# BattleZips/BattleZips-Halo2

Measured on AMD Instinct MI355X. Metric: complete proofs per second (synthesis + create_proof), BoardCircuit, k=14, IPA/Pasta, higher is better.
Workload: dtype u32x8 (255-bit modular integer, Montgomery)

## Files before the change

### battlezips-halo2_amd/bzh2/__init__.py

```python
from __future__ import annotations

import ctypes
import os

import numpy as np

_PKG = os.path.dirname(os.path.abspath(__file__))
_LIB_PATH = os.path.join(os.path.dirname(_PKG), "libbzh2.so")

OK, E_ARG, E_OOM, E_HIP, E_RANGE, E_NOGPU = 0, -1, -2, -3, -4, -5
CURVE_VESTA, CURVE_PALLAS, CURVE_BN254 = 0, 1, 2
FIELD_FP, FIELD_FQ, FIELD_BN254_FR, FIELD_BN254_FQ = 0, 1, 2, 3
FORM_CANONICAL, FORM_MONTGOMERY = 0, 1
MEM_HOST, MEM_DEVICE = 0, 1
T_MSM_DIGITS, T_MSM_ACCUMULATE, T_MSM_REDUCE, T_MSM_FINALIZE, T_NTT, T_COUNT = 0, 1, 2, 3, 4, 8
TIMER_NAMES = {0: "msm_digits", 1: "msm_accumulate", 2: "msm_reduce", 3: "msm_finalize", 4: "ntt"}

CURVE_SCALAR_FIELD = {CURVE_VESTA: FIELD_FP, CURVE_PALLAS: FIELD_FQ, CURVE_BN254: FIELD_BN254_FR}

EXPORTS = [
    "bzh_version", "bzh_strerror", "bzh_device_count", "bzh_ctx_create", "bzh_ctx_create_on_stream",
    "bzh_ctx_destroy", "bzh_ctx_sync", "bzh_last_error", "bzh_ctx_profile", "bzh_ctx_timings", "bzh_ctx_work", "bzh_ctx_msm_additions",
    "bzh_bases_upload", "bzh_bases_precompute", "bzh_bases_free", "bzh_bases_len", "bzh_bases_walk", "bzh_bases_points", "bzh_msm", "bzh_ntt", "bzh_coeff_to_extended",
    "bzh_jacobian_to_affine", "bzh_jacobian_sum", "bzh_affine_compress", "bzh_field_omega",
# ... 439 lines not shown
    out = np.zeros((v.shape[0], half, 4), dtype=np.uint64)
    _bind_poly(load())
    rc = load().bzh_fold(self.handle, field, _vp(v), half, v.shape[0], _vp(u), u.shape[0], form, MEM_HOST, _vp(out))
    self._check(rc, "bzh_fold")
    return out


def _ctx_vec_mul(self, field: int, a, b, form: int = FORM_CANONICAL) -> np.ndarray:
    a, b = _as_elems(a).copy(), _as_elems(b)
    _bind_poly(load())
    self._check(load().bzh_vec_mul(self.handle, field, _vp(a), _vp(b), a.size // 4, form, MEM_HOST), "bzh_vec_mul")
    return a


Context.batch_invert = _ctx_batch_invert
Context.prefix_product = _ctx_prefix_product
Context.eval_polynomial = _ctx_eval_polynomial
Context.inner_product = _ctx_inner_product
Context.fold = _ctx_fold
Context.vec_mul = _ctx_vec_mul


EXPORTS += ["bzh_pk_quotient_select", "bzh_pk_quotient_selected", "bzh_quotient_source_for_circuit", "bzh_builtin_quotients",
            "bzh_quotient_degree_histogram", "bzh_pk_lookup_select", "bzh_pk_lookup_selected"]
EXPORTS += ["bzh_record_stride", "bzh_record_encode", "bzh_record_decode", "bzh_record_to_json", "bzh_record_from_json"]
EXPORTS += ["bzh_transcript_new", "bzh_transcript_free", "bzh_transcript_common_point", "bzh_transcript_common_scalar",
            "bzh_transcript_write_point", "bzh_transcript_write_scalar", "bzh_transcript_squeeze_challenge",
            "bzh_transcript_proof"]


class Transcript:

    def __init__(self, challenge_field: int = FIELD_FP):
        L = load()
        vp = ctypes.c_void_p
        L.bzh_transcript_new.argtypes = [ctypes.c_int, ctypes.POINTER(vp)]
        for f in ("bzh_transcript_free",):
            getattr(L, f).argtypes = [vp]
        for f in ("bzh_transcript_common_point", "bzh_transcript_common_scalar", "bzh_transcript_write_scalar",
                  "bzh_transcript_squeeze_challenge"):
            getattr(L, f).argtypes = [vp, ctypes.POINTER(ctypes.c_uint64)]
        L.bzh_transcript_write_point.argtypes = [vp, ctypes.c_int, ctypes.POINTER(ctypes.c_uint64)]
        L.bzh_transcript_proof.argtypes = [vp, ctypes.POINTER(ctypes.POINTER(ctypes.c_uint8)), ctypes.POINTER(ctypes.c_size_t)]
        self.h = vp()
        rc = L.bzh_transcript_new(challenge_field, ctypes.byref(self.h))
        if rc != OK:
            raise BzhError(rc, "bzh_transcript_new")
# ... 262 lines not shown
```

### battlezips-halo2_amd/bzh2/native.py

```python
from __future__ import annotations

import ctypes

import numpy as np

from . import CURVE_SCALAR_FIELD, FORM_CANONICAL, FORM_MONTGOMERY, MEM_DEVICE, MEM_HOST, Bases, BzhError, Context, int_to_limbs, load
from .circuit_data import MODULI, Circuit, serialize_circuit

_VP = ctypes.c_void_p


def _bind():
    L = load()
    if getattr(L, "_bzh_native_bound", False):
        return L
    L.bzh_pk_create.argtypes = [_VP, _VP, ctypes.c_char_p, ctypes.c_size_t, ctypes.POINTER(_VP)]
    L.bzh_pk_free.argtypes = [_VP, _VP]
    L.bzh_pk_set_lagrange.argtypes = [_VP, _VP]
    L.bzh_pk_info.argtypes = [_VP, ctypes.POINTER(ctypes.c_size_t), ctypes.POINTER(ctypes.c_size_t), ctypes.POINTER(ctypes.c_uint32),
                              ctypes.POINTER(ctypes.c_uint32), ctypes.POINTER(ctypes.c_uint32)]
    L.bzh_verify_batch.argtypes = [_VP, _VP, ctypes.c_size_t, _VP, ctypes.c_size_t, _VP, ctypes.c_size_t, ctypes.POINTER(ctypes.c_size_t), _VP,
                                   ctypes.POINTER(ctypes.c_int)]
    L.bzh_prove_batch.argtypes = [_VP, _VP, ctypes.c_size_t, _VP, ctypes.c_int, ctypes.c_int, _VP, ctypes.c_size_t, ctypes.c_char_p,
                                  ctypes.c_size_t, _VP, ctypes.c_size_t, ctypes.POINTER(ctypes.c_size_t)]
# ... 100 lines not shown
                                                          np.concatenate([int_to_limbs(wp[0]), int_to_limbs(wp[1])])]))
        blob = bytes(circuit) if isinstance(circuit, (bytes, bytearray)) else serialize_circuit(circuit, self.p, vk_repr)
        L = _bind()
        h = _VP()
        ctx._check(L.bzh_pk_create(ctx.handle, self.bases.handle, blob, len(blob), ctypes.byref(h)), "bzh_pk_create")
        self.handle = h
        rb, mp = ctypes.c_size_t(), ctypes.c_size_t()
        na, nr, ur = ctypes.c_uint32(), ctypes.c_uint32(), ctypes.c_uint32()
        ctx._check(L.bzh_pk_info(h, ctypes.byref(rb), ctypes.byref(mp), ctypes.byref(na), ctypes.byref(nr), ctypes.byref(ur)), "bzh_pk_info")
        self.rng_bytes, self.max_proof_bytes, self.num_advice, self.n, self.usable_rows = rb.value, mp.value, na.value, nr.value, ur.value
        if params is not None:
            self.set_lagrange(params.bases_lagrange)

    def vk_repr(self):
        out, ph = (ctypes.c_uint8 * 32)(), ctypes.c_int()
        self.ctx._check(_bind().bzh_pk_vk_repr(self.handle, out, ctypes.byref(ph)), "bzh_pk_vk_repr")
        return int.from_bytes(bytes(out), "little"), bool(ph.value)

    def quotient_stats(self) -> dict:
        L = _bind()
        L.bzh_pk_quotient_stats.argtypes = [_VP] + [ctypes.POINTER(ctypes.c_uint32)] * 4
        v = [ctypes.c_uint32() for _ in range(4)]
        self.ctx._check(L.bzh_pk_quotient_stats(self.handle, *[ctypes.byref(x) for x in v]), "bzh_pk_quotient_stats")
        return {"ops": v[0].value, "multiplications_per_row": v[1].value, "lds_slots": v[2].value, "hoisted_columns": v[3].value}

    def quotient_source(self) -> str:
        L = _bind()
        L.bzh_pk_quotient_source.argtypes = [_VP, ctypes.c_char_p, ctypes.c_size_t, ctypes.POINTER(ctypes.c_size_t)]
        n = ctypes.c_size_t()
        self.ctx._check(L.bzh_pk_quotient_source(self.handle, None, 0, ctypes.byref(n)), "bzh_pk_quotient_source")
        buf = ctypes.create_string_buffer(n.value + 1)
        self.ctx._check(L.bzh_pk_quotient_source(self.handle, buf, n.value + 1, ctypes.byref(n)), "bzh_pk_quotient_source")
        return buf.value.decode()

    def set_quotient_module(self, code_object: bytes | None):
        L = _bind()
        L.bzh_pk_set_quotient_module.argtypes = [_VP, _VP, ctypes.c_char_p, ctypes.c_size_t]
        self.ctx._check(L.bzh_pk_set_quotient_module(self.ctx.handle, self.handle, code_object, len(code_object) if code_object else 0),
                        "bzh_pk_set_quotient_module")

    def quotient_selected(self):
        L = _bind()
        L.bzh_pk_quotient_selected.argtypes = [_VP, ctypes.POINTER(ctypes.c_int), ctypes.POINTER(ctypes.c_int)]
        f, b = ctypes.c_int(), ctypes.c_int()
        self.ctx._check(L.bzh_pk_quotient_selected(self.handle, ctypes.byref(f), ctypes.byref(b)), "bzh_pk_quotient_selected")
        return f.value, bool(b.value)

# ... 205 lines not shown
```

### battlezips-halo2_amd/csrc/exprvm.hip

```cpp
#include "ctx.hpp"
#include "field.cuh"
#include "host_field.hpp"

namespace bzh {

static constexpr int kExprSlots = 24;

struct ExprOp {
    uint8_t op, dst, a_kind, b_kind;
    int32_t a_idx, b_idx, a_rot, b_rot;
};

template <class P>
__device__ __forceinline__ Fe<P> expr_operand(int kind, int idx, int rot, const Fe<P>* slots, const uint32_t* const* cols,
                                               const size_t* strides, const uint32_t* consts, size_t r, size_t mask, size_t v) {
    if (kind == BZH_EXPR_SLOT) return slots[idx];
    if (kind == BZH_EXPR_CONST) return fe_load<P>(consts + (size_t)idx * 8);
    const size_t row = (r + (size_t)(int64_t)rot) & mask;
    return fe_load<P>(cols[idx] + (v * strides[idx] + row) * 8);
}

template <class P>
__global__ void __launch_bounds__(256) k_expr_eval(const ExprOp* __restrict__ prog, int nops, const uint32_t* const* __restrict__ cols,
                                                     const size_t* __restrict__ strides, const uint32_t* __restrict__ consts,
// ... 86 lines not shown
    else
        hipLaunchKernelGGL((k_expr_eval<P>), grid, block, 0, ctx->stream, d_prog, nops, d_cols, d_strides, d_consts, const_stride, size,
                           result_slot, d_out);
    BZH_HIP_TRY(ctx, hipGetLastError());
    return BZH_OK;
}

int expr_eval(bzh_ctx* ctx, int field, const void* d_prog, int nops, const uint32_t* const* d_cols, const size_t* d_strides,
              const uint32_t* d_consts, size_t const_stride, size_t size, int result_slot, size_t batch, int nslots, uint32_t* d_out) {
    const ExprOp* p = (const ExprOp*)d_prog;
    return with_field(field, [&](auto f) {
        return expr_eval_t<decltype(f)>(ctx, p, nops, d_cols, d_strides, d_consts, const_stride, size, result_slot, batch, nslots, d_out);
    });
}


struct ExprOp2 {
    uint8_t code, a_kind, b_kind, pad;
    int32_t a_idx, b_idx;
    int16_t a_rot, b_rot;
};
static_assert(sizeof(ExprOp2) == 16, "ExprOp2 layout");

static constexpr int kVm2Threads = 128;

template <class P>
__global__ void __launch_bounds__(kVm2Threads) k_expr_vm2(const ExprOp2* __restrict__ prog, int nops, const uint32_t* const* __restrict__ cols,
                                                           const size_t* __restrict__ strides, const uint32_t* __restrict__ consts,
                                                           size_t const_stride, size_t size, uint32_t* __restrict__ out) {
    extern __shared__ uint4 vm2_lds[];
    const size_t r = blockIdx.x * (size_t)kVm2Threads + threadIdx.x, v = blockIdx.y;
    if (r >= size) return;
    const size_t mask = size - 1;
    const uint32_t* cv = consts + v * const_stride * 8;
    const unsigned t = threadIdx.x;
    Fe<P> r0 = fe_zero<P>(), r1 = r0, r2 = r0, r3 = r0;
    auto leaf = [&](int kind, int idx, int rot) -> Fe<P> {
        if (kind == BZH_EXPR_COLUMN) {
            const size_t row = (r + (size_t)(int64_t)rot) & mask;
            return fe_load<P>(cols[idx] + (v * strides[idx] + row) * 8);
        }
        if (kind == BZH_EXPR_CONST) return fe_load<P>(cv + (size_t)idx * 8);
        Fe<P> x;
        const uint4 lo = vm2_lds[((size_t)idx * 2) * kVm2Threads + t], hi = vm2_lds[((size_t)idx * 2 + 1) * kVm2Threads + t];
        x.l[0] = lo.x, x.l[1] = lo.y, x.l[2] = lo.z, x.l[3] = lo.w, x.l[4] = hi.x, x.l[5] = hi.y, x.l[6] = hi.z, x.l[7] = hi.w;
        return x;
    };
    auto store = [&](int idx, const Fe<P>& x) {
        vm2_lds[((size_t)idx * 2) * kVm2Threads + t] = make_uint4(x.l[0], x.l[1], x.l[2], x.l[3]);
        vm2_lds[((size_t)idx * 2 + 1) * kVm2Threads + t] = make_uint4(x.l[4], x.l[5], x.l[6], x.l[7]);
    };
#define VM2_ARITH(OP, A, B) ((OP) == 0 ? fe_add(A, B) : ((OP) == 1 ? fe_sub(A, B) : ((OP) == 2 ? fe_mul(A, B) : fe_sub(B, A))))
#define VM2_SS(OP, P0, RA, RB) case (0 << 4) | ((OP) << 2) | (P0): RA = VM2_ARITH(OP, RA, RB); break;
#define VM2_SL(OP, P0, RA)     case (1 << 4) | ((OP) << 2) | (P0): { const Fe<P> b_ = leaf(op.b_kind, op.b_idx, op.b_rot); RA = VM2_ARITH(OP, RA, b_); } break;
#define VM2_LL(OP, P0, RA)     case (2 << 4) | ((OP) << 2) | (P0): { const Fe<P> a_ = leaf(op.a_kind, op.a_idx, op.a_rot); const Fe<P> b_ = leaf(op.b_kind, op.b_idx, op.b_rot); RA = VM2_ARITH(OP, a_, b_); } break;
#define VM2_ALLOPS_SS(P0, RA, RB) VM2_SS(0, P0, RA, RB) VM2_SS(1, P0, RA, RB) VM2_SS(2, P0, RA, RB) VM2_SS(3, P0, RA, RB)
#define VM2_ALLOPS_SL(P0, RA) VM2_SL(0, P0, RA) VM2_SL(1, P0, RA) VM2_SL(2, P0, RA) VM2_SL(3, P0, RA)
#define VM2_ALLOPS_LL(P0, RA) VM2_LL(0, P0, RA) VM2_LL(1, P0, RA) VM2_LL(2, P0, RA)
#define VM2_UN(P0, RA)                                                                                   \
    case (3 << 4) | (0 << 2) | (P0): RA = fe_neg(RA); break;                                              \
    case (3 << 4) | (1 << 2) | (P0): RA = leaf(op.a_kind, op.a_idx, op.a_rot); break;                     \
    case (3 << 4) | (2 << 2) | (P0): store(op.a_idx, RA); break;
    ExprOp2 nxt = prog[0];
    for (int i = 0; i < nops; i++) {
        const ExprOp2 op = nxt;
        nxt = prog[i + 1 < nops ? i + 1 : i];
        switch (op.code) {
            VM2_ALLOPS_SS(0, r0, r1) VM2_ALLOPS_SS(1, r1, r2) VM2_ALLOPS_SS(2, r2, r3)
            VM2_ALLOPS_SL(0, r0) VM2_ALLOPS_SL(1, r1) VM2_ALLOPS_SL(2, r2) VM2_ALLOPS_SL(3, r3)
            VM2_ALLOPS_LL(0, r0) VM2_ALLOPS_LL(1, r1) VM2_ALLOPS_LL(2, r2) VM2_ALLOPS_LL(3, r3)
            VM2_UN(0, r0) VM2_UN(1, r1) VM2_UN(2, r2) VM2_UN(3, r3)
            default: break;
        }
    }
#undef VM2_UN
#undef VM2_ALLOPS_LL
#undef VM2_ALLOPS_SL
#undef VM2_ALLOPS_SS
#undef VM2_LL
#undef VM2_SL
#undef VM2_SS
#undef VM2_ARITH
    fe_store(out + (v * size + r) * 8, r0);
}

int expr_eval2(bzh_ctx* ctx, int field, const void* d_prog, int nops, const uint32_t* const* d_cols, const size_t* d_strides,
               const uint32_t* d_consts, size_t const_stride, size_t size, size_t batch, int nlds, uint32_t* d_out) {
    if (size % kVm2Threads) return BZH_E_ARG;
    const size_t lds = (size_t)std::max(nlds, 1) * 2 * kVm2Threads * sizeof(uint4);
    if (lds > 64 * 1024) return BZH_E_RANGE;
    ScopedTimer t(ctx, BZH_T_QUOTIENT);
    const dim3 grid((unsigned)(size / kVm2Threads), (unsigned)batch), block(kVm2Threads);
    const ExprOp2* p = (const ExprOp2*)d_prog;
    BZH_TRY(with_pasta_field(field, [&](auto f) {
        hipLaunchKernelGGL((k_expr_vm2<decltype(f)>), grid, block, lds, ctx->stream, p, nops, d_cols, d_strides, d_consts, const_stride, size, d_out);
        return BZH_OK;
    }));
    BZH_HIP_TRY(ctx, hipGetLastError());
    return BZH_OK;
}

int expr_slots() { return kExprSlots; }

}
```

### battlezips-halo2_amd/csrc/prove.hip

```cpp
#include <algorithm>
#include <chrono>
#include <cstdio>
#include <cstdlib>
#include <cstring>
#include <map>
#include <set>
#include <memory>
#include <string>
#include <thread>
#include <vector>

#include "chacha.hpp"
#include "ctx.hpp"
#include "curve.cuh"
#include "fe29.cuh"
#include "host_field.hpp"

extern "C" const bzh_builtin_quotient* bzh_builtin_quotients(size_t* count) __attribute__((weak));

#include "prove_kernels.cuh"
#include "key_shape.hpp"
#include "quotient_program.hpp"
#include "proving_key.hpp"
#include "verifying_key.hpp"
// ... 163 lines not shown
    if (!pk) return BZH_E_ARG;
    if (g_lagrange && ((g_lagrange->n != pk->n + 2 && g_lagrange->n != pk->n + 3) || g_lagrange->curve != pk->curve || g_lagrange->device != pk->device || !g_lagrange->pre_c))
        return BZH_E_ARG;
    std::lock_guard<std::mutex> lk(pk->mu);
    pk->srs_lagrange = g_lagrange;
    return BZH_OK;
}

int bzh_pk_quotient_stats(bzh_pk* pk, uint32_t* ops, uint32_t* multiplications, uint32_t* lds_slots, uint32_t* hoisted_columns) {
    if (!pk) return BZH_E_ARG;
    uint32_t no = 0, nm = 0, nl = 0;
    if (pk->q_ok) {
        no = (uint32_t)pk->qprog.ops.size();
        nl = (uint32_t)pk->qprog.nlds;
        for (auto& o : pk->qprog.ops) nm += ((o.code >> 4) < 3 && ((o.code >> 2) & 3) == bzh::V2_MUL);
    }
    if (ops) *ops = no;
    if (multiplications) *multiplications = nm;
    if (lds_slots) *lds_slots = nl;
    if (hoisted_columns) *hoisted_columns = (uint32_t)pk->hoist_cols;
    return BZH_OK;
}

static int copy_text(const std::string& src, char* buf, size_t cap, size_t* len) {
    *len = src.size();
    if (buf && cap) {
        const size_t n = std::min(cap - 1, src.size());
        memcpy(buf, src.data(), n);
        buf[n] = 0;
    }
    return BZH_OK;
}

int bzh_pk_quotient_source(bzh_pk* pk, char* buf, size_t cap, size_t* len) {
    if (!pk || !len) return BZH_E_ARG;
    if (!pk->q_ok) return BZH_E_RANGE;
    return copy_text(bzh::program2_source(pk->qprog, pk->field), buf, cap, len);
}

int bzh_quotient_source_for_circuit(int curve, const uint8_t* circuit, size_t circuit_len, char* buf, size_t cap, size_t* len,
                                    uint64_t* program_hash) {
    if (!circuit || !len) return BZH_E_ARG;
    bzh_pk pk;
    BZH_TRY(bzh::with_pasta_curve(curve, [&](auto c) {
        using C = decltype(c);
        bzh::ParsedKey<typename bzh::CurveInfo<C>::SF> po;
        return bzh::pk_parse_t<C>(circuit, circuit_len, pk, po);
    }));
    if (!pk.q_ok) return BZH_E_RANGE;
    if (program_hash) *program_hash = pk.q_hash;
    return copy_text(bzh::program2_source(pk.qprog, pk.field, true) + "\n" + bzh::program2_source29(pk.qprog, pk.field), buf, cap, len);
}

int bzh_quotient_degree_histogram(int curve, const uint8_t* circuit, size_t circuit_len, uint32_t* polys, uint32_t* muls) {
    if (!circuit || !polys || !muls) return BZH_E_ARG;
    return bzh::with_pasta_curve(curve, [&](auto c) { return quotient_histogram_t<decltype(c)>(circuit, circuit_len, polys, muls); });
}

int bzh_pk_quotient_select(bzh_pk* pk, int flavour) {
    if (!pk) return BZH_E_ARG;
    std::lock_guard<std::mutex> lk(pk->mu);
    switch (flavour) {
        case BZH_QUOTIENT_INTERPRETER: break;
        case BZH_QUOTIENT_BUILTIN:
            if (!pk->q_builtin) return BZH_E_RANGE;
            break;
        case BZH_QUOTIENT_MODULE:
            if (!pk->q_fn) return BZH_E_RANGE;
            break;
        default: return BZH_E_ARG;
    }
    pk->q_select = flavour;
    return BZH_OK;
}
// ... 241 lines not shown
```

### battlezips-halo2_amd/csrc/quotient_program.hpp

```cpp
#pragma once
enum { EX_CONST, EX_SYMBOL, EX_QUERY, EX_NEG, EX_ADD, EX_MUL, EX_SCALE };
struct ENode {
    uint8_t tag;
    int32_t col = 0, rot = 0;
    uint32_t val[8] = {0};
    int a = -1, b = -1;
};
enum { SY_THETA, SY_BETA, SY_GAMMA, SY_Y, SY_XN, SY_X1, SY_X2, SY_X4, SY_BD0  };

struct ConstEnt {
    int sym = -1;
    uint32_t val[8] = {0};
};
struct Program {
    std::vector<bzh_expr_op> ops;
    std::vector<ConstEnt> consts;
    int result_slot = 0;
};

struct EPool {
    std::vector<ENode> n;
    struct NodeKey {
        uint8_t tag;
        int32_t col, rot, a, b;
// ... 147 lines not shown
            a = operand(e.a);
        } else {
            a = operand(e.a);
            b = operand(e.b);
        }
        const int d = a.release >= 0 ? a.release : (b.release >= 0 ? b.release : alloc());
        push(e.tag == EX_ADD ? BZH_EXPR_ADD : BZH_EXPR_MUL, d, a, b);
        if (a.release >= 0 && a.release != d) free_slots.push_back(a.release);
        if (b.release >= 0 && b.release != d) free_slots.push_back(b.release);
        return d;
    }
};


struct ExprOp2 {
    uint8_t code, a_kind, b_kind, pad;
    int32_t a_idx, b_idx;
    int16_t a_rot, b_rot;
};
enum { BZH_EXPR_LDS = 3 };
enum { V2_ADD = 0, V2_SUB = 1, V2_MUL = 2, V2_RSUB = 3 };
enum { V2_SS = 0, V2_SL = 1, V2_LL = 2, V2_UN = 3, V2_NEG = 0, V2_LOAD = 1, V2_STORE = 2 };
static constexpr int kV2Regs = 4, kV2LdsAcc = 0, kV2LdsInner = 1, kV2LdsCse0 = 2, kV2LdsCseMax = 8, kV2LdsSpills = 2, kV2LdsGlobalMax = 6;
enum { SY_YPOW0 = 4096  };

struct Program2 {
    std::vector<ExprOp2> ops;
    std::vector<ConstEnt> consts;
    bool ok = true;
    int nlds = 2;
};

static uint64_t program2_hash(const Program2& pg, int field) {
    uint64_t h = 1469598103934665603ull;
    auto mix = [&](const void* p, size_t n) {
        for (size_t i = 0; i < n; i++) h = (h ^ ((const uint8_t*)p)[i]) * 1099511628211ull;
    };
    mix(&field, sizeof(field));
    mix(&pg.nlds, sizeof(pg.nlds));
    for (const ExprOp2& o : pg.ops) {
        const int32_t w[7] = {o.code, o.a_kind, o.a_idx, o.a_rot, o.b_kind, o.b_idx, o.b_rot};
        mix(w, sizeof(w));
    }
    return h;
}

static std::string program2_source(const Program2& pg, int field, bool builtin = false) {
    std::string src;
    char buf[512];
    auto add = [&](const char* fmt, auto... a) {
        snprintf(buf, sizeof(buf), fmt, a...);
        src += buf;
    };
    const unsigned long long hash = (unsigned long long)program2_hash(pg, field);
// ... 353 lines not shown
    add("}  // namespace bzh_q29_%016llx\n", hash);
    return src;
}
static std::string program2_source29(const Program2& pg, int field) {
    int pa = 0, pb = 0;
    const std::string a = program2_source29_policy(pg, field, true, &pa), b = program2_source29_policy(pg, field, false, &pb);
    if (a.empty() || b.empty()) return a.empty() ? b : a;
    return pb < pa ? b : a;
}

struct Compiler2 {
    const EPool& pool;
    Program2 prog;
    int depth = 0;
    std::map<int, int> cse;
    std::map<int, int> hoisted;
    std::vector<int> label;
    int spill_used = 0, cse_slots = 6, max_lds = kV2LdsInner;
    struct GlobalEnt {
        int slot, first, last;
    };
    int global_slots = 6;
    std::map<int, GlobalEnt> gsel;
    explicit Compiler2(const EPool& p) : pool(p), label(p.n.size(), -1) {
        if (const char* e = getenv("BZH_VM2_CSE")) cse_slots = std::max(0, std::min(kV2LdsCseMax, atoi(e)));
        if (const char* e = getenv("BZH_VM2_GLOBAL")) global_slots = std::max(0, std::min(kV2LdsGlobalMax, atoi(e)));
    }
    int nlds() const { return max_lds + 1; }

    struct Leaf {
        int kind, idx, rot;
    };
    int const_index(int sym, const uint32_t* val) {
        for (size_t i = 0; i < prog.consts.size(); i++) {
            const ConstEnt& c = prog.consts[i];
            if (sym >= 0 ? c.sym == sym : (c.sym < 0 && !memcmp(c.val, val, 32))) return (int)i;
        }
        ConstEnt c;
        c.sym = sym;
        if (sym < 0) memcpy(c.val, val, 32);
        prog.consts.push_back(c);
        return (int)prog.consts.size() - 1;
    }
    bool is_leaf(int i) const {
        const ENode& e = pool.n[i];
        return e.tag == EX_CONST || e.tag == EX_SYMBOL || e.tag == EX_QUERY || cse.count(i) || hoisted.count(i);
    }
    Leaf leaf_of(int i) {
        auto ih = hoisted.find(i);
        if (ih != hoisted.end()) return {BZH_EXPR_COLUMN, ih->second, 0};
        auto it = cse.find(i);
        if (it != cse.end()) return {BZH_EXPR_LDS, it->second, 0};
        const ENode& e = pool.n[i];
        if (e.tag == EX_CONST) return {BZH_EXPR_CONST, const_index(-1, e.val), 0};
        if (e.tag == EX_SYMBOL) return {BZH_EXPR_CONST, const_index(e.col, nullptr), 0};
        if (e.rot < -32768 || e.rot > 32767) prog.ok = false;
        return {BZH_EXPR_COLUMN, e.col, e.rot};
    }
    int label_of(int i) {
        if (is_leaf(i)) return 0;
        if (label[i] >= 0) return label[i];
        const ENode& e = pool.n[i];
        int d;
        if (e.tag == EX_NEG || e.tag == EX_SCALE) d = std::max(1, label_of(e.a));
        else {
            const int la = label_of(e.a), lb = label_of(e.b);
            d = (la == 0 && lb == 0) ? 1 : (la == lb ? la + 1 : std::max(la, lb));
        }
        return label[i] = d;
    }
    void op(int form, int o, int pos, Leaf a = {0, 0, 0}, Leaf b = {0, 0, 0}) {
        if (pos < 0 || pos >= kV2Regs) prog.ok = false;
        ExprOp2 x;
        x.code = (uint8_t)((form << 4) | (o << 2) | (pos & 3));
        x.a_kind = (uint8_t)a.kind, x.b_kind = (uint8_t)b.kind, x.pad = 0;
        x.a_idx = a.idx, x.b_idx = b.idx;
        x.a_rot = (int16_t)a.rot, x.b_rot = (int16_t)b.rot;
        prog.ops.push_back(x);
    }
    bool is_plain_neg(int i) const { return pool.n[i].tag == EX_NEG && !cse.count(i); }
// ... 121 lines not shown
                int p = 0, o = 0;
                reach(kv.first, seen, chosen, &p, &o);
                if (p == 0) continue;
                const int first = kv.second.front(), last = kv.second.back();
                int slot = -1;
                for (int sl = 0; sl < global_slots && slot < 0; sl++) {
                    bool free_ = true;
                    for (auto& iv : busy[(size_t)sl]) free_ &= last < iv.first || first > iv.second;
                    if (free_) slot = sl;
                }
                if (slot < 0) continue;
                const double benefit = (double)(kv.second.size() - 1) * (200.0 * p + 25.0 * o) - 30.0;
                const double score = benefit / (double)(last - first + 1);
                if (benefit > 0 && score > best_score) best_score = score, best_n = kv.first, best_slot = slot;
            }
            if (best_n < 0) break;
            const std::vector<int>& gs = where[best_n];
            gsel[best_n] = GlobalEnt{base + best_slot, gs.front(), gs.back()};
            busy[(size_t)best_slot].push_back({gs.front(), gs.back()});
            chosen.insert(best_n);
            max_lds = std::max(max_lds, base + best_slot);
        }
    }
    std::set<int> gparked;
    void open_scope(const std::vector<int>& roots, int group = -1) {
        cse.clear();
        want.clear();
        for (auto& kv : gsel) {
            if (group < kv.second.first || group > kv.second.last) continue;
            if (gparked.count(kv.first)) cse[kv.first] = kv.second.slot;
            else want[kv.first] = kv.second.slot;
        }
        std::fill(label.begin(), label.end(), -1);
        std::map<int, int> uses, weight;
        for (int r : roots) count_uses(r, uses, weight);
        std::vector<std::pair<long, int>> cand;
        for (auto& kv : uses) {
            if (kv.second >= 2 && !gsel.count(kv.first)) cand.push_back({-(long)(kv.second - 1) * weight[kv.first], kv.first});
        }
        std::sort(cand.begin(), cand.end());
        for (size_t k = 0; k < cand.size() && k < (size_t)cse_slots; k++) {
            want[cand[k].second] = kV2LdsCse0 + (int)k;
            max_lds = std::max(max_lds, kV2LdsCse0 + (int)k);
        }
    }

// ... 33 lines not shown
                }
                for (auto& kv : uses) {
                    if (kv.second < 2 || where[kv.first].size() < 2) continue;
                    const ENode& e = pool.n[kv.first];
                    fprintf(stderr, "[vm2-shared] node %d tag %d weight %d uses %d groups", kv.first, (int)e.tag, weight[kv.first], kv.second);
                    for (int gi : where[kv.first]) fprintf(stderr, " %d", gi);
                    fprintf(stderr, "\n");
                }
            }
            fprintf(stderr, "[vm2] groups %zu, unique product nodes %zu, glue products (y powers, selectors, ACC) ~%zu, nodes used more than once %zu\n",
                    groups.size(), uniq_mul, horner, shared);
        }
        const Leaf y{BZH_EXPR_CONST, const_index(SY_Y, nullptr), 0};
        const Leaf acc{BZH_EXPR_LDS, kV2LdsAcc, 0}, inner{BZH_EXPR_LDS, kV2LdsInner, 0};
        {
            std::vector<std::vector<int>> group_roots;
            for (auto& g : groups) {
                group_roots.push_back(g.c);
                if (g.s >= 0) group_roots.back().push_back(g.s);
            }
            gparked.clear();
            select_globals(group_roots);
        }
        bool first_group = true;
        int group_index = -1;
        for (auto& g : groups) {
            group_index++;
            std::vector<int> roots = g.c;
            if (g.s >= 0) roots.push_back(g.s);
            open_scope(roots, group_index);
            const size_t m = g.c.size();
            if (m > 64) prog.ok = false;
            for (size_t j = 0; j < m; j++) {
                depth = 0;
                if (j == 0) {
                    emit(g.c[0]);
                } else if (label_of(g.c[j]) < kV2Regs) {
                    op(V2_LL, V2_MUL, 0, inner, y);
                    depth = 1;
                    emit(g.c[j]);
                    op(V2_SS, V2_ADD, 0);
                    depth = 1;
                } else {
                    emit(g.c[j]);
                    op(V2_LL, V2_MUL, 1, inner, y);
                    op(V2_SS, V2_ADD, 0);
                }
                if (j + 1 < m) op(V2_UN, V2_STORE, 0, inner);
            }
            if (g.s >= 0) {
                if (is_leaf(g.s)) {
                    op(V2_SL, V2_MUL, 0, Leaf{0, 0, 0}, leaf_of(g.s));
                } else if (label_of(g.s) < kV2Regs) {
                    depth = 1;
                    emit(g.s);
                    op(V2_SS, V2_MUL, 0);
                } else {
                    op(V2_UN, V2_STORE, 0, inner);
                    depth = 0;
                    emit(g.s);
                    op(V2_SL, V2_MUL, 0, Leaf{0, 0, 0}, inner);
                }
            }
            if (!first_group) {
                const Leaf ym{BZH_EXPR_CONST, const_index(m == 1 ? SY_Y : SY_YPOW0 + (int)m, nullptr), 0};
                op(V2_LL, V2_MUL, 1, acc, ym);
                op(V2_SS, V2_ADD, 0);
            }
            op(V2_UN, V2_STORE, 0, acc);
            first_group = false;
        }
        cse.clear();
        want.clear();
        op(V2_SL, V2_MUL, 0, Leaf{0, 0, 0}, leaf_of(tinv_node));
    }
};

struct Cols {
    std::vector<const uint32_t*> ptr;
    std::vector<size_t> stride;
    std::map<uint64_t, int> index;
    int add(uint64_t key, const uint32_t* p, size_t s) {
        auto it = index.find(key);
        if (it != index.end()) return it->second;
        const int i = (int)ptr.size();
        index[key] = i;
        ptr.push_back(p);
        stride.push_back(s);
        return i;
    }
    int at(uint64_t key) const { return index.at(key); }
};
```

### include/bzh2.h

```cpp
#ifndef BZH2_H
#define BZH2_H

#include <stddef.h>
#include <stdint.h>

#ifdef __cplusplus
extern "C" {
#endif

typedef struct bzh_ctx bzh_ctx;
typedef struct bzh_bases bzh_bases;
typedef struct bzh_transcript bzh_transcript;

typedef enum {
    BZH_OK = 0,
    BZH_E_ARG = -1,
    BZH_E_OOM = -2,
    BZH_E_HIP = -3,
    BZH_E_RANGE = -4,
    BZH_E_NOGPU = -5,
    BZH_E_VERIFY = -6
} bzh_status;

typedef enum { BZH_CURVE_VESTA = 0, BZH_CURVE_PALLAS = 1, BZH_CURVE_BN254 = 2 } bzh_curve;
// ... 86 lines not shown
                  const uint64_t* consts, size_t nconsts, unsigned log_size, int result_slot, int form, int mem, uint64_t* out);

int bzh_expr_eval_batch(bzh_ctx* ctx, int field, const bzh_expr_op* prog, size_t nops, const uint64_t* const* columns,
                        const size_t* column_strides, size_t ncols, const uint64_t* consts, size_t nconsts, size_t const_stride,
                        unsigned log_size, int result_slot, size_t batch, int form, int mem, uint64_t* out);

int bzh_ipa_open(bzh_ctx* ctx, const bzh_bases* bases, const uint64_t* poly, int form, int mem, const uint64_t* blind,
                 const uint64_t* x3, const uint8_t* rng, size_t rng_len, bzh_transcript* transcript, uint64_t* out_v);
int bzh_ipa_open_batch(bzh_ctx* ctx, const bzh_bases* bases, const uint64_t* polys, int form, int mem, size_t batch,
                       const uint64_t* blinds, const uint64_t* x3s, const uint8_t* rng, size_t rng_stride,
                       bzh_transcript* const* transcripts, uint64_t* out_v);
int bzh_ipa_verify(bzh_ctx* ctx, const bzh_bases* bases, const uint64_t* commitment_xy, const uint64_t* x3, const uint64_t* v,
                   const uint8_t* proof, size_t proof_len, bzh_transcript* transcript, const uint64_t* g0_u_w);

typedef struct bzh_pk bzh_pk;
#define BZH_CIRCUIT_BLOB_VK_REPR_OFFSET 24
#define BZH_VK_REPR_PLACEHOLDER 0x1234
int bzh_vk_digest(const char* pinned_debug, size_t len, uint8_t* out_repr32);
int bzh_pk_vk_repr(const bzh_pk* pk, uint8_t* out_repr32, int* is_placeholder);
int bzh_pk_create(bzh_ctx* ctx, const bzh_bases* srs, const uint8_t* circuit, size_t circuit_len, bzh_pk** out);
int bzh_pk_free(bzh_ctx* ctx, bzh_pk* pk);
int bzh_pk_set_lagrange(bzh_pk* pk, const bzh_bases* g_lagrange);
int bzh_pk_quotient_stats(bzh_pk* pk, uint32_t* ops, uint32_t* multiplications, uint32_t* lds_slots, uint32_t* hoisted_columns);
typedef enum { BZH_QUOTIENT_INTERPRETER = 0, BZH_QUOTIENT_BUILTIN = 1, BZH_QUOTIENT_MODULE = 2 } bzh_quotient_flavour;
int bzh_pk_quotient_source(bzh_pk* pk, char* buf, size_t cap, size_t* len);
int bzh_pk_set_quotient_module(bzh_ctx* ctx, bzh_pk* pk, const void* code_object, size_t len);
int bzh_pk_quotient_select(bzh_pk* pk, int flavour);
int bzh_pk_quotient_selected(bzh_pk* pk, int* flavour, int* builtin_available);
typedef enum { BZH_LOOKUP_HOST = 0, BZH_LOOKUP_DEVICE = 1 } bzh_lookup_where;
int bzh_pk_lookup_select(bzh_pk* pk, int where);
int bzh_pk_lookup_selected(bzh_pk* pk, int* where);
typedef enum { BZH_VERIFY_POINTS_HOST = 0, BZH_VERIFY_POINTS_DEVICE = 1 } bzh_verify_points_where;
int bzh_pk_verify_select(bzh_pk* pk, int where);
int bzh_pk_verify_selected(bzh_pk* pk, int* where);
int bzh_quotient_source_for_circuit(int curve, const uint8_t* circuit, size_t circuit_len, char* buf, size_t cap, size_t* len,
                                    uint64_t* program_hash);
int bzh_quotient_degree_histogram(int curve, const uint8_t* circuit, size_t circuit_len, uint32_t* polys16, uint32_t* muls16);
typedef void (*bzh_quotient_launch_fn)(unsigned grid_x, unsigned grid_y, void* hip_stream, const uint32_t* const* cols, const size_t* strides,
                                       const uint32_t* consts, size_t const_stride, size_t size, uint32_t* out);
typedef struct { uint64_t program_hash; bzh_quotient_launch_fn launch; const char* name; bzh_quotient_launch_fn launch29; } bzh_builtin_quotient;
const bzh_builtin_quotient* bzh_builtin_quotients(size_t* count);
int bzh_pk_info(const bzh_pk* pk, size_t* rng_bytes_per_proof, size_t* max_proof_bytes, uint32_t* num_advice, uint32_t* n_rows,
                uint32_t* usable_rows);
int bzh_verify_batch(bzh_ctx* ctx, bzh_pk* pk, size_t batch, const uint64_t* instances, size_t instance_rows, const uint8_t* proofs,
                     size_t proof_stride, const size_t* proof_lens, const uint64_t* g0_u_w, int* results);
int bzh_prove_batch(bzh_ctx* ctx, bzh_pk* pk, size_t batch, const uint64_t* advice, int form, int mem, const uint64_t* instances,
                    size_t instance_rows, const uint8_t* rng, size_t rng_stride, uint8_t* proofs, size_t proof_stride,
                    size_t* proof_lens);

typedef struct bzh_vk bzh_vk;
int bzh_vk_create(bzh_ctx* ctx, const bzh_bases* srs, const uint8_t* circuit, size_t circuit_len, bzh_vk** out);
int bzh_vk_from_pk(bzh_ctx* ctx, bzh_pk* pk, bzh_vk** out);
int bzh_vk_write(const bzh_vk* vk, uint8_t* out, size_t cap, size_t* len);
int bzh_vk_read(const uint8_t* bytes, size_t len, bzh_vk** out);
int bzh_vk_info(const bzh_vk* vk, int* curve, unsigned* k, uint32_t* num_instance, uint32_t* num_fixed_commitments,
                uint32_t* num_permutation_commitments, size_t* max_proof_bytes);
int bzh_vk_vk_repr(const bzh_vk* vk, uint8_t* out_repr32, int* is_placeholder);
int bzh_vk_device_bytes(const bzh_vk* vk, size_t* key_bytes, size_t* workspace_bytes);
int bzh_pk_device_bytes(const bzh_pk* pk, size_t* key_bytes, size_t* workspace_bytes);
// ... 83 lines not shown
```

Measured before the change: 740.8.

## Cache reused quotient column leaves in LDS across expression groups

The quotient-program compiler now picks column queries that are loaded several times across consecutive constraint groups. It loads each one once into dedicated LDS leaf slots, and later uses read from LDS instead of global memory. The change is meant to cut repeated global loads per row in the quotient VM. More LDS per row lowers occupancy, so the kernel gains a 64-thread variant for cases where 128 threads would exceed 64 KiB. It also adds introspection APIs for load counts and the compiled program.

```diff
diff --git a/battlezips-halo2_amd/bzh2/__init__.py b/battlezips-halo2_amd/bzh2/__init__.py
--- a/battlezips-halo2_amd/bzh2/__init__.py
+++ b/battlezips-halo2_amd/bzh2/__init__.py
@@ -485,7 +485,8 @@
 
 
 EXPORTS += ["bzh_pk_quotient_select", "bzh_pk_quotient_selected", "bzh_quotient_source_for_circuit", "bzh_builtin_quotients",
-            "bzh_quotient_degree_histogram", "bzh_pk_lookup_select", "bzh_pk_lookup_selected"]
+            "bzh_quotient_degree_histogram", "bzh_pk_lookup_select", "bzh_pk_lookup_selected", "bzh_pk_quotient_loads",
+            "bzh_quotient_program_for_circuit"]
 EXPORTS += ["bzh_record_stride", "bzh_record_encode", "bzh_record_decode", "bzh_record_to_json", "bzh_record_from_json"]
 EXPORTS += ["bzh_transcript_new", "bzh_transcript_free", "bzh_transcript_common_point", "bzh_transcript_common_scalar",
             "bzh_transcript_write_point", "bzh_transcript_write_scalar", "bzh_transcript_squeeze_challenge",
diff --git a/battlezips-halo2_amd/bzh2/native.py b/battlezips-halo2_amd/bzh2/native.py
--- a/battlezips-halo2_amd/bzh2/native.py
+++ b/battlezips-halo2_amd/bzh2/native.py
@@ -146,7 +146,11 @@
         L.bzh_pk_quotient_stats.argtypes = [_VP] + [ctypes.POINTER(ctypes.c_uint32)] * 4
         v = [ctypes.c_uint32() for _ in range(4)]
         self.ctx._check(L.bzh_pk_quotient_stats(self.handle, *[ctypes.byref(x) for x in v]), "bzh_pk_quotient_stats")
-        return {"ops": v[0].value, "multiplications_per_row": v[1].value, "lds_slots": v[2].value, "hoisted_columns": v[3].value}
+        L.bzh_pk_quotient_loads.argtypes = [_VP] + [ctypes.POINTER(ctypes.c_uint32)] * 2
+        w = [ctypes.c_uint32() for _ in range(2)]
+        self.ctx._check(L.bzh_pk_quotient_loads(self.handle, *[ctypes.byref(x) for x in w]), "bzh_pk_quotient_loads")
+        return {"ops": v[0].value, "multiplications_per_row": v[1].value, "lds_slots": v[2].value, "hoisted_columns": v[3].value,
+                "loads_per_row": w[0].value, "leaf_slots": w[1].value}
 
     def quotient_source(self) -> str:
         L = _bind()
diff --git a/battlezips-halo2_amd/csrc/exprvm.hip b/battlezips-halo2_amd/csrc/exprvm.hip
--- a/battlezips-halo2_amd/csrc/exprvm.hip
+++ b/battlezips-halo2_amd/csrc/exprvm.hip
@@ -132,14 +132,14 @@
 };
 static_assert(sizeof(ExprOp2) == 16, "ExprOp2 layout");
 
-static constexpr int kVm2Threads = 128;
-
-template <class P>
-__global__ void __launch_bounds__(kVm2Threads) k_expr_vm2(const ExprOp2* __restrict__ prog, int nops, const uint32_t* const* __restrict__ cols,
+static constexpr int kVm2Threads = 128, kVm2ThreadsSmall = 64;
+
+template <class P, int kRows>
+__global__ void __launch_bounds__(kRows) k_expr_vm2(const ExprOp2* __restrict__ prog, int nops, const uint32_t* const* __restrict__ cols,
                                                            const size_t* __restrict__ strides, const uint32_t* __restrict__ consts,
                                                            size_t const_stride, size_t size, uint32_t* __restrict__ out) {
     extern __shared__ uint4 vm2_lds[];
-    const size_t r = blockIdx.x * (size_t)kVm2Threads + threadIdx.x, v = blockIdx.y;
+    const size_t r = blockIdx.x * (size_t)kRows + threadIdx.x, v = blockIdx.y;
     if (r >= size) return;
     const size_t mask = size - 1;
     const uint32_t* cv = consts + v * const_stride * 8;
@@ -152,13 +152,13 @@
         }
         if (kind == BZH_EXPR_CONST) return fe_load<P>(cv + (size_t)idx * 8);
         Fe<P> x;
-        const uint4 lo = vm2_lds[((size_t)idx * 2) * kVm2Threads + t], hi = vm2_lds[((size_t)idx * 2 + 1) * kVm2Threads + t];
+        const uint4 lo = vm2_lds[((size_t)idx * 2) * kRows + t], hi = vm2_lds[((size_t)idx * 2 + 1) * kRows + t];
         x.l[0] = lo.x, x.l[1] = lo.y, x.l[2] = lo.z, x.l[3] = lo.w, x.l[4] = hi.x, x.l[5] = hi.y, x.l[6] = hi.z, x.l[7] = hi.w;
         return x;
     };
     auto store = [&](int idx, const Fe<P>& x) {
-        vm2_lds[((size_t)idx * 2) * kVm2Threads + t] = make_uint4(x.l[0], x.l[1], x.l[2], x.l[3]);
-        vm2_lds[((size_t)idx * 2 + 1) * kVm2Threads + t] = make_uint4(x.l[4], x.l[5], x.l[6], x.l[7]);
+        vm2_lds[((size_t)idx * 2) * kRows + t] = make_uint4(x.l[0], x.l[1], x.l[2], x.l[3]);
+        vm2_lds[((size_t)idx * 2 + 1) * kRows + t] = make_uint4(x.l[4], x.l[5], x.l[6], x.l[7]);
     };
 #define VM2_ARITH(OP, A, B) ((OP) == 0 ? fe_add(A, B) : ((OP) == 1 ? fe_sub(A, B) : ((OP) == 2 ? fe_mul(A, B) : fe_sub(B, A))))
 #define VM2_SS(OP, P0, RA, RB) case (0 << 4) | ((OP) << 2) | (P0): RA = VM2_ARITH(OP, RA, RB); break;
@@ -197,13 +197,18 @@
 int expr_eval2(bzh_ctx* ctx, int field, const void* d_prog, int nops, const uint32_t* const* d_cols, const size_t* d_strides,
                const uint32_t* d_consts, size_t const_stride, size_t size, size_t batch, int nlds, uint32_t* d_out) {
     if (size % kVm2Threads) return BZH_E_ARG;
-    const size_t lds = (size_t)std::max(nlds, 1) * 2 * kVm2Threads * sizeof(uint4);
+    const size_t per_row = (size_t)std::max(nlds, 1) * 2 * sizeof(uint4);
+    const int threads = per_row * kVm2Threads <= 64 * 1024 ? kVm2Threads : kVm2ThreadsSmall;
+    const size_t lds = per_row * (size_t)threads;
     if (lds > 64 * 1024) return BZH_E_RANGE;
     ScopedTimer t(ctx, BZH_T_QUOTIENT);
-    const dim3 grid((unsigned)(size / kVm2Threads), (unsigned)batch), block(kVm2Threads);
+    const dim3 grid((unsigned)(size / (size_t)threads), (unsigned)batch), block((unsigned)threads);
     const ExprOp2* p = (const ExprOp2*)d_prog;
     BZH_TRY(with_pasta_field(field, [&](auto f) {
-        hipLaunchKernelGGL((k_expr_vm2<decltype(f)>), grid, block, lds, ctx->stream, p, nops, d_cols, d_strides, d_consts, const_stride, size, d_out);
+        if (threads == kVm2Threads)
+            hipLaunchKernelGGL((k_expr_vm2<decltype(f), kVm2Threads>), grid, block, lds, ctx->stream, p, nops, d_cols, d_strides, d_consts, const_stride, size, d_out);
+        else
+            hipLaunchKernelGGL((k_expr_vm2<decltype(f), kVm2ThreadsSmall>), grid, block, lds, ctx->stream, p, nops, d_cols, d_strides, d_consts, const_stride, size, d_out);
         return BZH_OK;
     }));
     BZH_HIP_TRY(ctx, hipGetLastError());
diff --git a/battlezips-halo2_amd/csrc/prove.hip b/battlezips-halo2_amd/csrc/prove.hip
--- a/battlezips-halo2_amd/csrc/prove.hip
+++ b/battlezips-halo2_amd/csrc/prove.hip
@@ -209,6 +209,13 @@
     return BZH_OK;
 }
 
+int bzh_pk_quotient_loads(bzh_pk* pk, uint32_t* loads_per_row, uint32_t* leaf_slots) {
+    if (!pk) return BZH_E_ARG;
+    if (loads_per_row) *loads_per_row = pk->q_ok ? (uint32_t)bzh::program2_loads(pk->qprog) : 0;
+    if (leaf_slots) *leaf_slots = pk->q_ok ? (uint32_t)pk->qprog.leaf_slots : 0;
+    return BZH_OK;
+}
+
 static int copy_text(const std::string& src, char* buf, size_t cap, size_t* len) {
     *len = src.size();
     if (buf && cap) {
@@ -237,6 +244,41 @@
     if (!pk.q_ok) return BZH_E_RANGE;
     if (program_hash) *program_hash = pk.q_hash;
     return copy_text(bzh::program2_source(pk.qprog, pk.field, true) + "\n" + bzh::program2_source29(pk.qprog, pk.field), buf, cap, len);
+}
+
+int bzh_quotient_program_for_circuit(int curve, const uint8_t* circuit, size_t circuit_len, void* ops, size_t ops_cap, size_t* nops,
+                                     void* consts, size_t consts_cap, size_t* nconsts, uint32_t* stats8) {
+    if (!circuit || !nops || !nconsts) return BZH_E_ARG;
+    bzh_pk pk;
+    BZH_TRY(bzh::with_pasta_curve(curve, [&](auto c) {
+        using C = decltype(c);
+        bzh::ParsedKey<typename bzh::CurveInfo<C>::SF> po;
+        return bzh::pk_parse_t<C>(circuit, circuit_len, pk, po);
+    }));
+    if (!pk.q_ok) return BZH_E_RANGE;
+    const bzh::Program2& pg = pk.qprog;
+    *nops = pg.ops.size();
+    *nconsts = pg.consts.size();
+    if (stats8) {
+        uint32_t nm = 0;
+        for (auto& o : pg.ops) nm += ((o.code >> 4) < 3 && ((o.code >> 2) & 3) == bzh::V2_MUL);
+        const uint32_t st[8] = {(uint32_t)pg.ops.size(), nm, (uint32_t)pg.nlds, (uint32_t)bzh::program2_loads(pg), (uint32_t)pg.leaf_slots,
+                                (uint32_t)pg.leaf_base, (uint32_t)pk.hoist_cols, 0};
+        memcpy(stats8, st, sizeof(st));
+    }
+    if (ops) {
+        if (ops_cap < pg.ops.size() * sizeof(bzh::ExprOp2)) return BZH_E_ARG;
+        memcpy(ops, pg.ops.data(), pg.ops.size() * sizeof(bzh::ExprOp2));
+    }
+    if (consts) {
+        if (consts_cap < pg.consts.size() * 40) return BZH_E_ARG;
+        for (size_t i = 0; i < pg.consts.size(); i++) {
+            uint32_t w[10] = {(uint32_t)pg.consts[i].sym, 0};
+            memcpy(w + 2, pg.consts[i].val, 32);
+            memcpy((uint8_t*)consts + 40 * i, w, 40);
+        }
+    }
+    return BZH_OK;
 }
 
 int bzh_quotient_degree_histogram(int curve, const uint8_t* circuit, size_t circuit_len, uint32_t* polys, uint32_t* muls) {
diff --git a/battlezips-halo2_amd/csrc/quotient_program.hpp b/battlezips-halo2_amd/csrc/quotient_program.hpp
--- a/battlezips-halo2_amd/csrc/quotient_program.hpp
+++ b/battlezips-halo2_amd/csrc/quotient_program.hpp
@@ -193,6 +193,8 @@
 enum { V2_ADD = 0, V2_SUB = 1, V2_MUL = 2, V2_RSUB = 3 };
 enum { V2_SS = 0, V2_SL = 1, V2_LL = 2, V2_UN = 3, V2_NEG = 0, V2_LOAD = 1, V2_STORE = 2 };
 static constexpr int kV2Regs = 4, kV2LdsAcc = 0, kV2LdsInner = 1, kV2LdsCse0 = 2, kV2LdsCseMax = 8, kV2LdsSpills = 2, kV2LdsGlobalMax = 6;
+static constexpr int kV2LdsLeafMax = 8, kV2LdsLeafDefault = 3;
+static constexpr char kV2LeafEnv[] = "BZH_VM2_LEAF";
 enum { SY_YPOW0 = 4096  };
 
 struct Program2 {
@@ -200,7 +202,17 @@
     std::vector<ConstEnt> consts;
     bool ok = true;
     int nlds = 2;
+    int leaf_base = 0, leaf_slots = 0;
 };
+static size_t program2_loads(const Program2& pg) {
+    size_t n = 0;
+    for (const ExprOp2& o : pg.ops) {
+        const int form = o.code >> 4, op = (o.code >> 2) & 3;
+        n += (form == V2_LL || (form == V2_UN && op == V2_LOAD)) && o.a_kind == BZH_EXPR_COLUMN;
+        n += (form == V2_SL || form == V2_LL) && o.b_kind == BZH_EXPR_COLUMN;
+    }
+    return n;
+}
 
 static uint64_t program2_hash(const Program2& pg, int field) {
     uint64_t h = 1469598103934665603ull;
@@ -600,10 +612,17 @@
     };
     int global_slots = 6;
     std::map<int, GlobalEnt> gsel;
+    struct LeafEnt {
+        int col, rot, slot, first, last;
+    };
+    int leaf_slots = kV2LdsLeafDefault, cur_group = -1;
+    std::vector<LeafEnt> lsel;
     explicit Compiler2(const EPool& p) : pool(p), label(p.n.size(), -1) {
         if (const char* e = getenv("BZH_VM2_CSE")) cse_slots = std::max(0, std::min(kV2LdsCseMax, atoi(e)));
         if (const char* e = getenv("BZH_VM2_GLOBAL")) global_slots = std::max(0, std::min(kV2LdsGlobalMax, atoi(e)));
-    }
+        if (const char* e = getenv(kV2LeafEnv)) leaf_slots = std::max(0, std::min(kV2LdsLeafMax, atoi(e)));
+    }
+    int leaf_base() const { return kV2LdsCse0 + cse_slots + kV2LdsSpills + global_slots; }
     int nlds() const { return max_lds + 1; }
 
     struct Leaf {
@@ -624,16 +643,21 @@
         const ENode& e = pool.n[i];
         return e.tag == EX_CONST || e.tag == EX_SYMBOL || e.tag == EX_QUERY || cse.count(i) || hoisted.count(i);
     }
+    Leaf column_leaf(int col, int rot) const {
+        for (const LeafEnt& l : lsel)
+            if (l.col == col && l.rot == rot && l.first <= cur_group && cur_group <= l.last) return {BZH_EXPR_LDS, l.slot, 0};
+        return {BZH_EXPR_COLUMN, col, rot};
+    }
     Leaf leaf_of(int i) {
         auto ih = hoisted.find(i);
-        if (ih != hoisted.end()) return {BZH_EXPR_COLUMN, ih->second, 0};
+        if (ih != hoisted.end()) return column_leaf(ih->second, 0);
         auto it = cse.find(i);
         if (it != cse.end()) return {BZH_EXPR_LDS, it->second, 0};
         const ENode& e = pool.n[i];
         if (e.tag == EX_CONST) return {BZH_EXPR_CONST, const_index(-1, e.val), 0};
         if (e.tag == EX_SYMBOL) return {BZH_EXPR_CONST, const_index(e.col, nullptr), 0};
         if (e.rot < -32768 || e.rot > 32767) prog.ok = false;
-        return {BZH_EXPR_COLUMN, e.col, e.rot};
+        return column_leaf(e.col, e.rot);
     }
     int label_of(int i) {
         if (is_leaf(i)) return 0;
@@ -801,6 +825,62 @@
             max_lds = std::max(max_lds, base + best_slot);
         }
     }
+    void select_leaves(const std::vector<int>& group_of, int ngroups) {
+        lsel.clear();
+        if (leaf_slots <= 0 || ngroups <= 0) return;
+        std::map<std::pair<int, int>, std::vector<int>> uses;
+        auto count = [&](int kind, int col, int rot, int g) {
+            if (kind != BZH_EXPR_COLUMN) return;
+            std::vector<int>& u = uses[{col, rot}];
+            if (u.empty()) u.assign((size_t)ngroups, 0);
+            u[(size_t)g]++;
+        };
+        for (size_t i = 0; i < prog.ops.size(); i++) {
+            const ExprOp2& o = prog.ops[i];
+            const int form = o.code >> 4, oo = (o.code >> 2) & 3;
+            if (form == V2_LL || (form == V2_UN && oo == V2_LOAD)) count(o.a_kind, o.a_idx, o.a_rot, group_of[i]);
+            if (form == V2_SL || form == V2_LL) count(o.b_kind, o.b_idx, o.b_rot, group_of[i]);
+        }
+        std::vector<std::vector<char>> busy((size_t)leaf_slots, std::vector<char>((size_t)ngroups, 0));
+        for (;;) {
+            double best_score = 0;
+            int best_saving = 0, best_slot = -1, best_first = 0, best_last = 0;
+            std::pair<int, int> best_leaf{0, 0};
+            for (auto& kv : uses) {
+                const std::vector<int>& u = kv.second;
+                for (int first = 0; first < ngroups; first++) {
+                    if (!u[(size_t)first]) continue;
+                    int loads = 0;
+                    unsigned free_ = (1u << leaf_slots) - 1;
+                    for (int last = first; last < ngroups && free_; last++) {
+                        for (int sl = 0; sl < leaf_slots; sl++)
+                            if (busy[(size_t)sl][(size_t)last]) free_ &= ~(1u << sl);
+                        if (!free_) break;
+                        if (!u[(size_t)last]) continue;
+                        loads += u[(size_t)last];
+                        const int saving = loads - 1;
+                        const double score = (double)saving / (double)(last - first + 1);
+                        if (saving > 0 && (score > best_score || (score == best_score && saving > best_saving))) {
+                            best_score = score, best_saving = saving, best_leaf = kv.first, best_first = first, best_last = last;
+                            best_slot = __builtin_ctz(free_);
+                        }
+                    }
+                }
+            }
+            if (best_slot < 0) break;
+            lsel.push_back(LeafEnt{best_leaf.first, best_leaf.second, leaf_base() + best_slot, best_first, best_last});
+            std::vector<int>& u = uses[best_leaf];
+            for (int g = best_first; g <= best_last; g++) busy[(size_t)best_slot][(size_t)g] = 1, u[(size_t)g] = 0;
+        }
+    }
+    void fill_leaves(int group) {
+        for (const LeafEnt& l : lsel) {
+            if (l.first != group) continue;
+            op(V2_UN, V2_LOAD, 0, Leaf{BZH_EXPR_COLUMN, l.col, l.rot});
+            op(V2_UN, V2_STORE, 0, Leaf{BZH_EXPR_LDS, l.slot, 0});
+            max_lds = std::max(max_lds, l.slot);
+        }
+    }
     std::set<int> gparked;
     void open_scope(const std::vector<int>& roots, int group = -1) {
         cse.clear();
@@ -880,57 +960,77 @@
             gparked.clear();
             select_globals(group_roots);
         }
-        bool first_group = true;
-        int group_index = -1;
-        for (auto& g : groups) {
-            group_index++;
-            std::vector<int> roots = g.c;
-            if (g.s >= 0) roots.push_back(g.s);
-            open_scope(roots, group_index);
-            const size_t m = g.c.size();
-            if (m > 64) prog.ok = false;
-            for (size_t j = 0; j < m; j++) {
-                depth = 0;
-                if (j == 0) {
-                    emit(g.c[0]);
-                } else if (label_of(g.c[j]) < kV2Regs) {
-                    op(V2_LL, V2_MUL, 0, inner, y);
-                    depth = 1;
-                    emit(g.c[j]);
-                    op(V2_SS, V2_ADD, 0);
-                    depth = 1;
-                } else {
-                    emit(g.c[j]);
-                    op(V2_LL, V2_MUL, 1, inner, y);
+        std::vector<int> group_of;
+        auto emit_groups = [&]() {
+            prog.ops.clear();
+            group_of.clear();
+            gparked.clear();
+            spill_used = 0;
+            bool first_group = true;
+            int group_index = -1;
+            for (auto& g : groups) {
+                group_index++;
+                cur_group = group_index;
+                std::vector<int> roots = g.c;
+                if (g.s >= 0) roots.push_back(g.s);
+                open_scope(roots, group_index);
+                fill_leaves(group_index);
+                const size_t m = g.c.size();
+                if (m > 64) prog.ok = false;
+                for (size_t j = 0; j < m; j++) {
+                    depth = 0;
+                    if (j == 0) {
+                        emit(g.c[0]);
+                    } else if (label_of(g.c[j]) < kV2Regs) {
+                        op(V2_LL, V2_MUL, 0, inner, y);
+                        depth = 1;
+                        emit(g.c[j]);
+                        op(V2_SS, V2_ADD, 0);
+                        depth = 1;
+                    } else {
+                        emit(g.c[j]);
+                        op(V2_LL, V2_MUL, 1, inner, y);
+                        op(V2_SS, V2_ADD, 0);
+                    }
+                    if (j + 1 < m) op(V2_UN, V2_STORE, 0, inner);
+                }
+                if (g.s >= 0) {
+                    if (is_leaf(g.s)) {
+                        op(V2_SL, V2_MUL, 0, Leaf{0, 0, 0}, leaf_of(g.s));
+                    } else if (label_of(g.s) < kV2Regs) {
+                        depth = 1;
+                        emit(g.s);
+                        op(V2_SS, V2_MUL, 0);
+                    } else {
+                        op(V2_UN, V2_STORE, 0, inner);
+                        depth = 0;
+                        emit(g.s);
+                        op(V2_SL, V2_MUL, 0, Leaf{0, 0, 0}, inner);
+                    }
+                }
+                if (!first_group) {
+                    const Leaf ym{BZH_EXPR_CONST, const_index(m == 1 ? SY_Y : SY_YPOW0 + (int)m, nullptr), 0};
+                    op(V2_LL, V2_MUL, 1, acc, ym);
                     op(V2_SS, V2_ADD, 0);
                 }
-                if (j + 1 < m) op(V2_UN, V2_STORE, 0, inner);
-            }
-            if (g.s >= 0) {
-                if (is_leaf(g.s)) {
-                    op(V2_SL, V2_MUL, 0, Leaf{0, 0, 0}, leaf_of(g.s));
-                } else if (label_of(g.s) < kV2Regs) {
-                    depth = 1;
-                    emit(g.s);
-                    op(V2_SS, V2_MUL, 0);
-                } else {
-                    op(V2_UN, V2_STORE, 0, inner);
-                    depth = 0;
-                    emit(g.s);
-                    op(V2_SL, V2_MUL, 0, Leaf{0, 0, 0}, inner);
-                }
-            }
-            if (!first_group) {
-                const Leaf ym{BZH_EXPR_CONST, const_index(m == 1 ? SY_Y : SY_YPOW0 + (int)m, nullptr), 0};
-                op(V2_LL, V2_MUL, 1, acc, ym);
-                op(V2_SS, V2_ADD, 0);
-            }
-            op(V2_UN, V2_STORE, 0, acc);
-            first_group = false;
-        }
-        cse.clear();
-        want.clear();
-        op(V2_SL, V2_MUL, 0, Leaf{0, 0, 0}, leaf_of(tinv_node));
+                op(V2_UN, V2_STORE, 0, acc);
+                first_group = false;
+                group_of.resize(prog.ops.size(), group_index);
+            }
+            cse.clear();
+            want.clear();
+            cur_group = -1;
+            op(V2_SL, V2_MUL, 0, Leaf{0, 0, 0}, leaf_of(tinv_node));
+            group_of.resize(prog.ops.size(), group_index);
+        };
+        emit_groups();
+        if (leaf_slots > 0 && prog.ok) {
+            select_leaves(group_of, (int)groups.size());
+            if (!lsel.empty()) emit_groups();
+        }
+        std::set<int> used;
+        for (const LeafEnt& l : lsel) used.insert(l.slot);
+        prog.leaf_base = leaf_base(), prog.leaf_slots = (int)used.size();
     }
 };
 
diff --git a/include/bzh2.h b/include/bzh2.h
--- a/include/bzh2.h
+++ b/include/bzh2.h
@@ -132,6 +132,7 @@
 int bzh_pk_free(bzh_ctx* ctx, bzh_pk* pk);
 int bzh_pk_set_lagrange(bzh_pk* pk, const bzh_bases* g_lagrange);
 int bzh_pk_quotient_stats(bzh_pk* pk, uint32_t* ops, uint32_t* multiplications, uint32_t* lds_slots, uint32_t* hoisted_columns);
+int bzh_pk_quotient_loads(bzh_pk* pk, uint32_t* loads_per_row, uint32_t* leaf_slots);
 typedef enum { BZH_QUOTIENT_INTERPRETER = 0, BZH_QUOTIENT_BUILTIN = 1, BZH_QUOTIENT_MODULE = 2 } bzh_quotient_flavour;
 int bzh_pk_quotient_source(bzh_pk* pk, char* buf, size_t cap, size_t* len);
 int bzh_pk_set_quotient_module(bzh_ctx* ctx, bzh_pk* pk, const void* code_object, size_t len);
@@ -145,6 +146,8 @@
 int bzh_pk_verify_selected(bzh_pk* pk, int* where);
 int bzh_quotient_source_for_circuit(int curve, const uint8_t* circuit, size_t circuit_len, char* buf, size_t cap, size_t* len,
                                     uint64_t* program_hash);
+int bzh_quotient_program_for_circuit(int curve, const uint8_t* circuit, size_t circuit_len, void* ops, size_t ops_cap, size_t* nops,
+                                     void* consts, size_t consts_cap, size_t* nconsts, uint32_t* stats8);
 int bzh_quotient_degree_histogram(int curve, const uint8_t* circuit, size_t circuit_len, uint32_t* polys16, uint32_t* muls16);
 typedef void (*bzh_quotient_launch_fn)(unsigned grid_x, unsigned grid_y, void* hip_stream, const uint32_t* const* cols, const size_t* strides,
                                        const uint32_t* consts, size_t const_stride, size_t size, uint32_t* out);
```

Measured after the change: 752.2 (median of 6 runs). 1.02x the previous value.
